# RazorClient/Stark-prover

Measured on AMD Instinct MI355X. Metric: FRI commit field-elems/sec at codeword 2^24; achieved HBM GB/s vs peak, higher is better.
Workload: dtype u32; 1 GPU; fri_commit codeword 2^24, blowup 8 (d=2^21), SHA-256 Merkle per layer, 21 rounds; codeword_log2=24, per_gpu_log2=24, blowup=8, field=p=3*2^30+1, parallelism=single GPU

## Files before the change

stark-prover_amd/csrc/fri_layer.hip:

```cpp
#include <cassert>
#include "fri_internal.hpp"
#include "sha256_fast.hpp"
#include "sha256_quad.hpp"

namespace fri {

#ifdef FRI_STAMPS
#define STAMP_WITH(on, i, fn)                                  \
    do {                                                       \
        if (on) t.st->stamps[t.k][(i)] = fn();                 \
    } while (0)
#else
#define STAMP_WITH(on, i, fn) do {} while (0)
#endif
#define STAMP(on, i) STAMP_WITH(on, i, __builtin_amdgcn_s_memrealtime)
#define STAMP_CLK(on, i) STAMP_WITH(on, i, __builtin_amdgcn_s_memtime)

#ifndef FRI_CHAIN_PRIO
#define FRI_CHAIN_PRIO 3
#endif
__device__ __forceinline__ void chain_prio() {
    if (FRI_CHAIN_PRIO > 0) __builtin_amdgcn_s_setprio(FRI_CHAIN_PRIO);
}

struct Dg { uint32_t w[8]; };

__device__ __forceinline__ void dg_load(const uint32_t* p, Dg& d) {
    uint4 a = reinterpret_cast<const uint4*>(p)[0], b = reinterpret_cast<const uint4*>(p)[1];
    d.w[0] = a.x; d.w[1] = a.y; d.w[2] = a.z; d.w[3] = a.w; d.w[4] = b.x; d.w[5] = b.y; d.w[6] = b.z; d.w[7] = b.w;
}
__device__ __forceinline__ void dg_store(uint32_t* p, const Dg& d) {
    reinterpret_cast<uint4*>(p)[0] = make_uint4(d.w[0], d.w[1], d.w[2], d.w[3]);
    reinterpret_cast<uint4*>(p)[1] = make_uint4(d.w[4], d.w[5], d.w[6], d.w[7]);
}
__device__ __forceinline__ void dg_lds_load(const uint4* p, Dg& d) {
    uint4 a = p[0], b = p[1];
    d.w[0] = a.x; d.w[1] = a.y; d.w[2] = a.z; d.w[3] = a.w; d.w[4] = b.x; d.w[5] = b.y; d.w[6] = b.z; d.w[7] = b.w;
}
__device__ __forceinline__ void dg_lds_store(uint4* p, const Dg& d) {
    p[0] = make_uint4(d.w[0], d.w[1], d.w[2], d.w[3]);
    p[1] = make_uint4(d.w[4], d.w[5], d.w[6], d.w[7]);
}
__device__ __forceinline__ void hnode(const Dg& l, const Dg& r, Dg& o) { shaf::node(l.w, r.w, o.w); }
__device__ __forceinline__ void hleaf(uint32_t v, Dg& o) { shaf::leaf(v, o.w); }
__device__ __forceinline__ void cnode(const Dg& l, const Dg& r, Dg& o) { shaf::node_compact(l.w, r.w, o.w); }
__device__ __forceinline__ void cleaf(uint32_t v, Dg& o) { shaf::leaf_compact(v, o.w); }

__device__ __forceinline__ void pair_level(const uint4* A, uint4* B, uint32_t* out, uint32_t tid, uint32_t cnt,
                                           const shaq::Role& R) {
    if (tid >= max(2 * cnt, 64u)) return;
    const uint32_t q = (tid >> 1) & (cnt - 1), half = (tid & 1u) ^ 1u;
    const bool real = tid < 2 * cnt;
    Dg a, b;
    dg_lds_load(A + 4 * q, a);
    dg_lds_load(A + 4 * q + 2, b);
    uint32_t o[4];
    shaq::node(a.w, b.w, o, R);
    if (!real) return;
    const uint4 v = make_uint4(o[0], o[1], o[2], o[3]);
    B[2 * q + half] = v;
    reinterpret_cast<uint4*>(out + 8 * q)[half] = v;
}

#ifndef FRI_SCHED_PRODUCER
#define FRI_SCHED_PRODUCER 1
#endif
struct SchedLds {
    uint32_t wk[32 * 48];
    uint32_t flag;
};
__device__ __forceinline__ void sched_init(SchedLds* sl) {
    if (FRI_SCHED_PRODUCER && threadIdx.x == 0) sl->flag = 0u;
}
__device__ __forceinline__ void pair_level_s(const uint4* A, uint4* B, uint32_t* out, uint32_t tid, uint32_t cnt,
                                             const shaq::Role& R, SchedLds* sl, uint32_t ord) {
    if (!FRI_SCHED_PRODUCER || cnt > 32) {
        pair_level(A, B, out, tid, cnt, R);
        return;
    }
    const uint32_t wv = tid >> 6;
    if (wv > 1) return;
    const uint32_t lane = tid & 63u;
    const uint32_t q = (lane >> 1) & (cnt - 1), half = (lane & 1u) ^ 1u;
    const bool real = lane < 2 * cnt;
    Dg a, b;
    dg_lds_load(A + 4 * q, a);
    dg_lds_load(A + 4 * q + 2, b);
    if (wv == 1) {
        uint32_t w[16];
#pragma unroll
        for (int i = 0; i < 8; i++) { w[i] = a.w[i]; w[8 + i] = b.w[i]; }
        shaq::produce(w, sl->wk + 48 * q, &sl->flag, 3u * ord, real && (lane & 1u) == 0u, lane == 0u, R);
        return;
    }
    uint32_t o[4];
    shaq::node_ext(a.w, b.w, o, R, sl->wk + 48 * q, &sl->flag, 3u * ord);
    if (!real) return;
    const uint4 v = make_uint4(o[0], o[1], o[2], o[3]);
    B[2 * q + half] = v;
    reinterpret_cast<uint4*>(out + 8 * q)[half] = v;
}

__device__ __forceinline__ void lds_barrier() {
    asm volatile("s_waitcnt lgkmcnt(0)\n\ts_barrier" ::: "memory");
}

__device__ __forceinline__ int wave_max_i(int v) {
#pragma unroll
    for (int off = 32; off > 0; off >>= 1) v = max(v, __shfl_xor(v, off));
    return v;
}

struct Mx3 {
    int m0 = -1, m1 = -1, m2 = -1;
    __device__ __forceinline__ void load(const int32_t* p, uint32_t i) { m0 = p[3 * i]; m1 = p[3 * i + 1]; m2 = p[3 * i + 2]; }
    __device__ __forceinline__ void take(const int32_t* p, uint32_t i) {
        m0 = max(m0, p[3 * i]); m1 = max(m1, p[3 * i + 1]); m2 = max(m2, p[3 * i + 2]);
    }
    __device__ __forceinline__ void store(int32_t* p, uint32_t i) const { p[3 * i] = m0; p[3 * i + 1] = m1; p[3 * i + 2] = m2; }
    __device__ __forceinline__ void wave_max() { m0 = wave_max_i(m0); m1 = wave_max_i(m1); m2 = wave_max_i(m2); }
};
__device__ __forceinline__ void mx3_wave_to_red(Mx3 m, int32_t* red, uint32_t tx) {
    m.wave_max();
    if ((tx & 63) == 0) m.store(red, tx >> 6);
}
__device__ __forceinline__ Mx3 mx3_from_red(const int32_t* red, uint32_t nw) {
    Mx3 m;
    for (uint32_t i = 0; i < nw; i++) m.take(red, i);
    return m;
}
struct Degree { int deg; bool noncanon; };
__device__ __forceinline__ Degree degree_of(int k, const Mx3& m) {
    return {k == 0 ? m.m0 : (m.m1 < 0 ? m.m2 : m.m0), k == 0 && m.m1 >= 0};
}

__device__ __forceinline__ void coef_slice(const LayerTask& t, uint32_t w, uint32_t G, int32_t* red, uint32_t t0,
                                           uint32_t nthr) {
    Mx3 m;
    const uint32_t tx = threadIdx.x - t0;
    const size_t jhi_all = t.jhi ? t.jhi : ~(size_t)0;
    if (t.k == 0) {
        const size_t a = t.jlo, b = min(t.d0, jhi_all), n = b > a ? b - a : 0;
        const size_t cs = (n + G - 1) / G, lo = a + (size_t)w * cs, hi = min(b, lo + cs);
        const uint32_t* in = t.coef_in - t.ibase;
        for (size_t j = lo + tx; j < hi; j += nthr) {
            const uint32_t c = in[j];
            if (c) m.m0 = max(m.m0, (int)j);
            if (c >= P) m.m1 = 0;
        }
    } else {
        const DevState* st = t.st;
        const size_t len = (size_t)(st->deg[t.k - 1] + 1), nlen = (len + 1) / 2;
        const uint32_t beta_m = st->beta_mont[t.k - 1];
        const size_t a = t.jlo, b = min(nlen, jhi_all), n = b > a ? b - a : 0;
        const size_t cs = (n + G - 1) / G, lo = a + (size_t)w * cs, hi = min(b, lo + cs);
        const uint32_t* in = t.coef_in - t.ibase;
        uint32_t* outp = t.coef_out - t.obase;
        for (size_t j = lo + tx; j < hi; j += nthr) {
            uint32_t e = in[2 * j];
            uint32_t o = (2 * j + 1 < len) ? in[2 * j + 1] : 0u;
            uint32_t v = add(e, mmul(o, beta_m));
            outp[j] = v;
            if (v) m.m0 = (int)j;
            if (e) m.m1 = (int)j;
            if (o) m.m2 = (int)j;
        }
    }
    mx3_wave_to_red(m, red, tx);
}
__device__ __forceinline__ void coef_combine(const LayerTask& t, uint32_t w, const int32_t* red, uint32_t nw) {
    mx3_from_red(red, nw).store(t.wgmax, w);
}
__device__ __forceinline__ void coef_task(const LayerTask& t, uint32_t w, uint32_t G, int32_t* red ) {
    coef_slice(t, w, G, red, 0, blockDim.x);
    lds_barrier();
    if (threadIdx.x == 0) coef_combine(t, w, red, blockDim.x / 64);
}

__device__ __forceinline__ void quad(const uint4& vals, uint32_t* lv0, uint32_t* lv1, size_t q ,
                                     Dg& out) {
    Dg a, b, c, d, n0, n1;
    hleaf(vals.x, a); hleaf(vals.y, b); hleaf(vals.z, c); hleaf(vals.w, d);
    dg_store(lv0 + 8 * (4 * q), a); dg_store(lv0 + 8 * (4 * q + 1), b);
    dg_store(lv0 + 8 * (4 * q + 2), c); dg_store(lv0 + 8 * (4 * q + 3), d);
    hnode(a, b, n0);
    hnode(c, d, n1);
    dg_store(lv1 + 8 * (2 * q), n0);
    dg_store(lv1 + 8 * (2 * q + 1), n1);
    hnode(n0, n1, out);
}

template <uint32_t TPB>
__device__ __forceinline__ void lds_two_levels(uint4* lds, const Dg& mine, uint32_t* lv2, uint32_t* lv3, uint32_t* lv4,
                                               size_t g2 ) {
    uint4* A = lds;
    uint4* B = lds + 2 * TPB;
    const uint32_t t = threadIdx.x;
    dg_store(lv2 + 8 * (g2 + t), mine);
    dg_lds_store(A + 2 * t, mine);
    lds_barrier();
    if (t < TPB / 2) {
        Dg l, r, o;
        dg_lds_load(A + 4 * t, l); dg_lds_load(A + 4 * t + 2, r);
        hnode(l, r, o);
        dg_lds_store(B + 2 * t, o);
        dg_store(lv3 + 8 * (g2 / 2 + t), o);
    }
    lds_barrier();
    if (t < TPB / 4) {
        Dg l, r, o;
        dg_lds_load(B + 4 * t, l); dg_lds_load(B + 4 * t + 2, r);
        hnode(l, r, o);
        dg_store(lv4 + 8 * (g2 / 4 + t), o);
    }
}

__device__ __forceinline__ bool gated_off(const LayerTask& t) {
    return t.gst && t.gidx >= 0 && !t.gst->active[t.gidx];
}

__device__ __forceinline__ uint32_t pair_beta(const LayerTask& t) { return t.gst->beta_mont[t.gidx]; }

template <bool FOLD, bool COMMIT, uint32_t TPB, bool PAIR = false>
__global__ __launch_bounds__(TPB) void k_layer_leaf(LayerTask t) {
    if (gated_off(t)) return;
    __shared__ uint4 lds[3 * TPB];
    __shared__ int32_t red[3 * (TPB / 64)];
    const uint32_t L = t.L;
    const size_t wg = PAIR ? (size_t)blockIdx.x + t.wg_base : (size_t)blockIdx.x;
    const size_t q = wg * TPB + threadIdx.x;
    uint4 v;
    if (FOLD) {
        const size_t half = (size_t)1 << L;
        const uint32_t beta_m = COMMIT ? t.st->beta_mont[t.k - 1] : (PAIR ? pair_beta(t) : t.beta_m);
        uint4 a = reinterpret_cast<const uint4*>(t.prev)[q];
        uint4 b = reinterpret_cast<const uint4*>(PAIR ? t.prev2 : t.prev + half)[q];
        uint4 x = reinterpret_cast<const uint4*>(t.xinv)[q];
        v.x = fold_one(a.x, b.x, x.x, beta_m); v.y = fold_one(a.y, b.y, x.y, beta_m);
        v.z = fold_one(a.z, b.z, x.z, beta_m); v.w = fold_one(a.w, b.w, x.w, beta_m);
        reinterpret_cast<uint4*>(t.values)[q] = v;
    } else {
        v = reinterpret_cast<const uint4*>(t.values)[q];
    }
    uint32_t* tr = t.tree;
    Dg top;
    quad(v, tr + 8 * level_offset(L, 0), tr + 8 * level_offset(L, 1), q, top);
    if (COMMIT) coef_task(t, blockIdx.x, gridDim.x, red);
    lds_two_levels<TPB>(lds, top, tr + 8 * level_offset(L, 2), tr + 8 * level_offset(L, 3),
                        tr + 8 * level_offset(L, 4), wg * TPB);
}

#ifndef WIDE_PAIR_MAX
#define WIDE_PAIR_MAX (1u << 16)
#endif

__host__ __device__ __forceinline__ uint32_t wide_levels(uint32_t L) { return L <= 8 + TOP_LOG ? 8u : 4u; }

template <bool FOLD, bool COMMIT, bool PAIR = false>
__global__ __launch_bounds__(256) void k_layer_leaf_wide(LayerTask t) {
    if (gated_off(t)) return;
    STAMP(COMMIT && blockIdx.x == 0 && threadIdx.x == 0, 60);
    __shared__ uint4 lds[2 * 256 + 2 * 128];
    __shared__ int32_t red[12];
    __shared__ SchedLds sl;
    sched_init(&sl);
    const uint32_t L = t.L;
    const size_t wg = PAIR ? (size_t)blockIdx.x + t.wg_base : (size_t)blockIdx.x;
    const size_t grid = PAIR ? (size_t)t.wg_total : (size_t)gridDim.x;
    const size_t i = wg * 256 + threadIdx.x;
    uint32_t v;
    if (FOLD) {
        const size_t half = (size_t)1 << L;
        const uint32_t beta_m = COMMIT ? t.st->beta_mont[t.k - 1] : (PAIR ? pair_beta(t) : t.beta_m);
        v = fold_one(t.prev[i], PAIR ? t.prev2[i] : t.prev[i + half], t.xinv[i], beta_m);
        t.values[i] = v;
    } else {
        v = t.values[i];
    }
    uint32_t* tr = t.tree;
    Dg d;
    cleaf(v, d);
    dg_store(tr + 8 * i, d);
    uint4* A = lds;
    uint4* B = lds + 2 * 256;
    dg_lds_store(A + 2 * threadIdx.x, d);
    lds_barrier();
    STAMP(COMMIT && blockIdx.x == 0 && threadIdx.x == 0, 61);
    uint32_t cnt = 256;
    const shaq::Role qr = shaq::role_of(threadIdx.x);
    if (grid * 128 < WIDE_PAIR_MAX) chain_prio();
    const uint32_t nlev = wide_levels(L);
#pragma unroll 1
    for (uint32_t j = 1; j <= nlev; j++) {
        cnt >>= 1;
        uint32_t* out = tr + 8 * (level_offset(L, j) + (wg << (8 - j)));
        if ((size_t)cnt * grid < WIDE_PAIR_MAX) {
            pair_level_s(A, B, out, threadIdx.x, cnt, qr, &sl, j);
        } else if (threadIdx.x < cnt) {
            Dg a, b, o;
            dg_lds_load(A + 4 * threadIdx.x, a);
            dg_lds_load(A + 4 * threadIdx.x + 2, b);
            hnode(a, b, o);
            dg_lds_store(B + 2 * threadIdx.x, o);
            dg_store(out + 8 * threadIdx.x, o);
        }
        if (COMMIT && j == 2 && threadIdx.x >= 128) coef_slice(t, blockIdx.x, gridDim.x, red, 128, 128);
        lds_barrier();
        uint4* tmp = A; A = B; B = tmp;
    }
    if (COMMIT && threadIdx.x == 128) coef_combine(t, blockIdx.x, red, 2);
    STAMP(COMMIT && blockIdx.x == 0 && threadIdx.x == 0, 62);
}

__device__ __forceinline__ void reduce_mx(const int32_t* in, int32_t* out, uint32_t w, uint32_t R) {
    if (threadIdx.x >= 64) return;
    Mx3 m;
    if (threadIdx.x < R) m.load(in, R * w + threadIdx.x);
    m.wave_max();
    if (threadIdx.x == 0) m.store(out, w);
}

__global__ __launch_bounds__(512) void k_tree_mid(uint32_t* tree, uint32_t L, uint32_t l, const DevState* st,
                                                  int gate, const int32_t* mx_in, int32_t* mx_out, uint32_t R) {
    if (st && gate >= 0 && !st->active[gate]) return;
    constexpr uint32_t NIN = 1024;
    __shared__ uint4 lds[NIN + NIN / 2];
    __shared__ SchedLds sl;
    sched_init(&sl);
    uint4* A = lds;
    uint4* B = lds + NIN;
    const uint32_t t = threadIdx.x;
    const size_t base = (size_t)blockIdx.x * NIN;
    const uint32_t* in = tree + 8 * level_offset(L, l);
    {
        Dg a, b, o;
        dg_load(in + 8 * (base + 2 * t), a);
        dg_load(in + 8 * (base + 2 * t + 1), b);
        if (mx_in) reduce_mx(mx_in, mx_out, blockIdx.x, R);
        hnode(a, b, o);
        dg_lds_store(A + 2 * t, o);
        dg_store(tree + 8 * (level_offset(L, l + 1) + (base >> 1) + t), o);
    }
    lds_barrier();
    const shaq::Role qr = shaq::role_of(t);
    uint32_t cnt = NIN / 2;
#pragma unroll 1
    for (uint32_t j = 2; j <= 4; j++) {
        cnt >>= 1;
        uint32_t* out = tree + 8 * (level_offset(L, l + j) + (base >> j));
        const bool narrow = (size_t)cnt * gridDim.x < WIDE_PAIR_MAX;
        if (narrow) {
            pair_level_s(A, B, out, t, cnt, qr, &sl, j);
        } else if (t < cnt) {
            Dg a, b, o;
            dg_lds_load(A + 4 * t, a);
            dg_lds_load(A + 4 * t + 2, b);
            hnode(a, b, o);
            dg_lds_store(B + 2 * t, o);
            dg_store(out + 8 * t, o);
        }
        lds_barrier();
        uint4* tmp = A; A = B; B = tmp;
    }
}

__global__ __launch_bounds__(256) void k_tree_mid8(uint32_t* tree, uint32_t L, uint32_t l, const DevState* st,
                                                   int gate, const int32_t* mx_in, int32_t* mx_out, uint32_t R) {
    if (st && gate >= 0 && !st->active[gate]) return;
    chain_prio();
    __shared__ uint4 lds[256 + 128];
    __shared__ SchedLds sl;
    sched_init(&sl);
    uint4* A = lds;
    uint4* B = lds + 256;
    const uint32_t t = threadIdx.x;
    const size_t base = (size_t)blockIdx.x * 256;
    const uint32_t* in = tree + 8 * level_offset(L, l);
    const shaq::Role qr = shaq::role_of(t);
    {
        const uint32_t q = t >> 1, half = (t & 1u) ^ 1u;
        Dg a, b;
        dg_load(in + 8 * (base + 2 * q), a);
        dg_load(in + 8 * (base + 2 * q + 1), b);
        if (mx_in) reduce_mx(mx_in, mx_out, blockIdx.x, R);
        uint32_t o[4];
        shaq::node(a.w, b.w, o, qr);
        const uint4 v = make_uint4(o[0], o[1], o[2], o[3]);
        A[2 * q + half] = v;
        reinterpret_cast<uint4*>(tree + 8 * (level_offset(L, l + 1) + (base >> 1) + q))[half] = v;
    }
    lds_barrier();
    uint32_t cnt = 128;
#pragma unroll 1
    for (uint32_t j = 2; j <= 8; j++) {
        cnt >>= 1;
        pair_level_s(A, B, tree + 8 * (level_offset(L, l + j) + (base >> j)), t, cnt, qr, &sl, j);
        lds_barrier();
        uint4* tmp = A; A = B; B = tmp;
    }
}

__device__ __forceinline__ void ktouch(const void* sym) {
    uint32_t a, b, c, d;
    asm volatile("s_nop 4\n\t"
                 "s_load_dword %0, %4, 0x0\n\ts_load_dword %1, %4, 0x40\n\t"
                 "s_load_dword %2, %4, 0x80\n\ts_load_dword %3, %4, 0xc0\n\t"
                 "s_waitcnt lgkmcnt(0)"
                 : "=&s"(a), "=&s"(b), "=&s"(c), "=&s"(d)
                 : "s"(sym)
                 : "memory");
}
__device__ __forceinline__ void kcache_touch_sha_tables() {
    ktouch(&shaf::KTAB[0]);
    ktouch(&shaf::PAD_KW_C.kw[0]);
    ktouch(&shaf::PAD_KW_1024.kw[0]);
    ktouch(&shaf::PAD_KW_1536.kw[0]);
}

__device__ __forceinline__ uint32_t hexch(uint32_t nib) { return nib < 10u ? 0x30u + nib : 0x57u + nib; }
__device__ __forceinline__ void hex2(uint32_t x, uint32_t& hi, uint32_t& lo) {
    hi = (hexch(x >> 28) << 24) | (hexch((x >> 24) & 15u) << 16) | (hexch((x >> 20) & 15u) << 8) | hexch((x >> 16) & 15u);
    lo = (hexch((x >> 12) & 15u) << 24) | (hexch((x >> 8) & 15u) << 16) | (hexch((x >> 4) & 15u) << 8) | hexch(x & 15u);
}
__device__ __forceinline__ uint32_t hexhex(uint32_t b) {
    const uint32_t x = ((b & 0xF0u) << 12) | (b & 0x0Fu);
    const uint32_t ge = ((x + 0x00060006u) >> 4) & 0x00010001u;
    return 0x33303330u + x + ge * 0x2F7u;
}

enum { CJ_REHASH = 0, CJ_MID = 2, CJ_ROOT = 3, CJ_FINAL = 6, CJ_END_ROUND = 6, CJ_END_FINAL = 8 };

__device__ __forceinline__ void chan_job(int j, uint32_t cs[8], uint32_t X[4], uint32_t has, const uint4* root_lds,
                                         uint32_t fv, const shaq::Role& R) {
    j = __builtin_amdgcn_readfirstlane(j);
    has = __builtin_amdgcn_readfirstlane(has);
    uint32_t w[16];
    const bool pad = (j == 1) || (j == 5);
    if (j == 0 || j == 2 || j == 6) {
#pragma unroll
        for (int i = 0; i < 8; i++) hex2(cs[i], w[2 * i], w[2 * i + 1]);
#pragma unroll
        for (int i = 0; i < 4; i++) X[i] = R.iv[i];
    } else if (j == 3 || j == 4) {
        const uint32_t b = (__lane_id() & 15u) + (j == 4 ? 16u : 0u);
        const uint32_t rw = reinterpret_cast<const uint32_t*>(root_lds)[b >> 2];
        const uint32_t hh = hexhex((rw >> (24 - 8 * (b & 3))) & 255u);
#pragma unroll
        for (int jj = 0; jj < 16; jj++) w[jj] = __builtin_amdgcn_readlane(hh, jj);
        if (j == 3 && !has) {
#pragma unroll
            for (int i = 0; i < 4; i++) X[i] = R.iv[i];
        }
    } else if (j == 7) {
#pragma unroll
        for (int i = 0; i < 16; i++) w[i] = 0u;
        w[0] = 0x30303030u; w[1] = 0x30303030u;
        hex2(fv, w[2], w[3]);
        w[4] = 0x80000000u;
        w[15] = 80u * 8u;
    }
    if (pad) shaq::compress_kw(X, j == 1 ? shaf::PAD_KW_C.kw : (has ? shaf::PAD_KW_1536.kw : shaf::PAD_KW_1024.kw), R);
    else shaq::compress(X, w, R);
    if (j == 1 || j == 5 || j == 7) {
#pragma unroll
        for (int i = 0; i < 4; i++) {
            const uint32_t o = shaq::swap01(X[i]);
            cs[i] = R.is_a ? X[i] : o;
            cs[4 + i] = R.is_a ? o : X[i];
        }
    }
}

constexpr uint32_t pow2_32k_mod_p(int k) {
    uint64_t r = 1;
    for (int j = 0; j < k; j++) r = (r << 32) % P;
    return (uint32_t)r;
}
__device__ __forceinline__ uint32_t chan_beta(const uint32_t s[8]) {
    constexpr uint32_t W[8] = {pow2_32k_mod_p(8), pow2_32k_mod_p(7), pow2_32k_mod_p(6), pow2_32k_mod_p(5),
                               pow2_32k_mod_p(4), pow2_32k_mod_p(3), pow2_32k_mod_p(2), pow2_32k_mod_p(1)};
    uint32_t t[8];
#pragma unroll
    for (int i = 0; i < 8; i++) t[i] = mmul(s[i] >= P ? s[i] - P : s[i], W[i]);
    return add(add(add(t[0], t[1]), add(t[2], t[3])), add(add(t[4], t[5]), add(t[6], t[7])));
}


template <typename Value>
__device__ __forceinline__ void leaf_loop(uint32_t N, uint32_t* tr, uint4* A, Value&& value) {
    for (uint32_t i = threadIdx.x; i < max(N, 64u); i += blockDim.x) {
        const uint32_t j = i & (N - 1);
        const bool real = i < N;
        const uint32_t v = value(j, real);
        Dg d;
        cleaf(v, d);
        if (real) {
            dg_store(tr + 8 * j, d);
            dg_lds_store(A + 2 * j, d);
        }
    }
}

__device__ __forceinline__ void level_step(const LayerTask& t, bool stamps, uint32_t it, const uint4* A, uint4* B,
                                           uint32_t* out, uint32_t cnt, const shaq::Role& R, SchedLds* sl,
                                           uint32_t ord) {
    const uint32_t tid = threadIdx.x;
    if (cnt <= 128) {
        STAMP_CLK(stamps && it < 18 && tid == 0, 24 + 2 * it);
        pair_level_s(A, B, out, tid, cnt, R, sl, ord);
        STAMP_CLK(stamps && it < 18 && tid == 0, 25 + 2 * it);
        return;
    }
#pragma unroll 1
    for (uint32_t q = tid; q < cnt; q += blockDim.x) {
        Dg a, b, o;
        dg_lds_load(A + 4 * q, a);
        dg_lds_load(A + 4 * q + 2, b);
#ifdef FRI_STAMPS
        if (stamps && it < 18 && q == 0) asm volatile("s_waitcnt lgkmcnt(0)" ::: "memory");
#endif
        STAMP_CLK(stamps && it < 18 && q == 0, 24 + 2 * it);
        cnode(a, b, o);
        STAMP_CLK(stamps && it < 18 && q == 0, 25 + 2 * it);
        dg_lds_store(B + 2 * q, o);
        dg_store(out + 8 * q, o);
    }
}

__device__ __forceinline__ int chan_drain(const LayerTask& t, int job, int job_end, bool level, uint32_t cnt,
                                           uint32_t cs[8], uint32_t X[4], uint32_t has, const uint4* root_lds,
                                           uint32_t fv, const shaq::Role& R) {
    if (job >= job_end || (level && !(cnt <= 192 && job < CJ_ROOT))) return job;
    do {
        STAMP(threadIdx.x == 448 && job == CJ_ROOT, 14);
        STAMP(threadIdx.x == 448 && job == CJ_ROOT + 2, 13);
        chan_job(job, cs, X, has, root_lds, fv, R);
        STAMP(threadIdx.x == 448 && job >= CJ_ROOT && job <= CJ_ROOT + 2, 20 + job - CJ_ROOT);
        job++;
    } while (!level && job < job_end);
    return job;
}

struct RoundOut { uint32_t active, beta_m; };
__device__ __forceinline__ RoundOut layer_results(const LayerTask& t, const Degree& dg, const uint32_t cs[8],
                                                  uint32_t fv, uint32_t fbeta1, const uint4* root_lds) {
    DevState* st = t.st;
    const int k = t.k, deg = dg.deg;
    if (dg.noncanon) {
        st->active[k] = 0;
        st->status = 1u;
        return {0u, 0u};
    }
    st->deg[k] = deg;
    Dg root;
    dg_lds_load(root_lds, root);
#pragma unroll
    for (int i = 0; i < 8; i++) st->roots[k][i] = root.w[i];
    st->n_layers = (uint32_t)k + 1;
    STAMP(true, 15);
    if (deg >= 1 && k < MAXR && t.L >= 1) {
        uint32_t beta = chan_beta(cs);
#pragma unroll
        for (int i = 0; i < 8; i++) st->chan[i] = cs[i];
        st->chan_has = 1;
        st->chan_pending = 1;
        if (fbeta1) beta = fbeta1 - 1u;
        st->beta[k] = beta;
        const uint32_t bm = to_mont(beta);
        st->beta_mont[k] = bm;
        st->active[k] = 1;
        st->n_rounds = (uint32_t)k + 1;
        STAMP(true, 16);
        return {1u, bm};
    }
    st->active[k] = 0;
    if (deg >= 1) { st->status = 7u; return {0u, 0u}; }
#pragma unroll
    for (int i = 0; i < 8; i++) st->chan[i] = cs[i];
    st->final_value = fv;
    st->final_degree = deg;
    st->chan_has = 1;
    st->chan_pending = 0;
    return {0u, 0u};
}

template <bool FROM_LEAVES, bool COMMIT, bool SHARD = false>
__global__ __launch_bounds__(512) void k_tree_top(LayerTask t, uint32_t l, const int32_t* mx, uint32_t G) {
    static_assert(!(FROM_LEAVES && (COMMIT || SHARD)), "from the leaves: standalone trees only");
    if (gated_off(t)) return;
    chain_prio();
    __shared__ uint4 lds[2 * 1024 + 2 * 512];
    __shared__ int32_t red[24];
    __shared__ SchedLds sl;
    sched_init(&sl);
    const uint32_t L = t.L;
    const uint32_t N = 1u << (L - l);
    const uint32_t tid = threadIdx.x;

    const bool chan_wave = COMMIT && tid >= 448;
    DevState* st = t.st;
    uint32_t cs[8], X[4];
    uint32_t has = 0, fbeta1 = 0;
    int job = CJ_END_FINAL;
    if (chan_wave) {
#pragma unroll
        for (int i = 0; i < 8; i++) cs[i] = st->chan[i];
        const uint32_t h = st->chan_has, pend = st->chan_pending;
        const uint32_t fo = COMMIT ? st->forced : 0u, fb = st->forced_beta[t.k < MAXR ? t.k : 0];
        has = h;
        job = !h ? CJ_ROOT : (pend ? CJ_REHASH : CJ_MID);
        if (fo && t.k < MAXR) fbeta1 = fb + 1u;
    }
    if (tid >= 384 && tid < 448) kcache_touch_sha_tables();
    uint4* A = lds;
    uint4* B = lds + 2 * 1024;
    uint32_t* tr = t.tree;
    STAMP(COMMIT && tid == 0, 0);
    if (FROM_LEAVES) {
        leaf_loop(N, tr, A, [&](uint32_t j, bool) { return t.values[j]; });
    } else if (SHARD && COMMIT) {
        const ShardTop& sh = *t.shard;
        for (uint32_t i = tid; i < N; i += blockDim.x) {
            Dg d;
            dg_load(sh.recs_in + REC_WORDS * sh.rank_of_block[i], d);
            dg_lds_store(A + 2 * i, d);
            dg_store(tr + 8 * i, d);
        }
        Mx3 m;
        if (tid < sh.G) {
            m.load(reinterpret_cast<const int32_t*>(sh.recs_in + REC_WORDS * tid + 8), 0);
            if (sh.sched_on) { m.m0 = sh.sched_deg; m.m1 = t.k == 0 ? -1 : 0; m.m2 = -1; }
        }
        mx3_wave_to_red(m, red, tid);
    } else {
        const uint32_t* in = tr + 8 * level_offset(L, l);
        Mx3 m;
        if (COMMIT && tid < G) m.load(mx, tid);
        for (uint32_t i = tid; i < N; i += blockDim.x) {
            Dg d;
            dg_load(in + 8 * i, d);
            dg_lds_store(A + 2 * i, d);
        }
        if (SHARD && !COMMIT) {
            const ShardTop& sh = *t.shard;
            for (uint32_t i = tid; i < sh.rec_R; i += blockDim.x) m.take(sh.rec_mx, i);
            mx3_wave_to_red(m, red, tid);
        }
        if (COMMIT) {
            for (uint32_t i = tid + blockDim.x; i < G; i += blockDim.x) m.take(mx, i);
            mx3_wave_to_red(m, red, tid);
        }
    }
    lds_barrier();
    const Degree dg = COMMIT ? degree_of(t.k, mx3_from_red(red, 8)) : Degree{-1, false};
    const bool is_final = COMMIT && dg.deg < 1;
    const int job_end = is_final ? CJ_END_FINAL : CJ_END_ROUND;
    uint32_t fv = 0;
    if (chan_wave && is_final && dg.deg == 0)
        fv = SHARD ? t.shard->recs_in[11] : (t.k == 0 ? t.coef_in : t.coef_out)[0];
    STAMP(COMMIT && tid == 0, 1);
    STAMP_CLK(COMMIT && tid == 0, 17);
    const uint32_t nlev = L - l;
    const uint32_t total = nlev + (COMMIT ? 1u : 0u);
    const shaq::Role R = shaq::role_of(tid);
    uint32_t cnt = N;
#pragma unroll 1
    for (uint32_t it = 0; it < total; it++) {
        const bool level = it < nlev;
        if (level) {
            cnt >>= 1;
            level_step(t, COMMIT, it, A, B, tr + 8 * level_offset(L, l + 1 + it), cnt, R, &sl, it);
        }
        if (chan_wave) job = chan_drain(t, job, job_end, level, cnt, cs, X, has, A, fv, R);
        lds_barrier();
        if (level) {
            uint4* tmp = A; A = B; B = tmp;
            STAMP(COMMIT && tid == 0 && it < 11, 2 + it);
            STAMP_CLK(COMMIT && tid == 0 && it + 1 == nlev, 18);
            STAMP(COMMIT && tid == 0 && it + 1 == nlev, 19);
        }
    }
    if (SHARD && !COMMIT && tid == 448) {
        const ShardTop& sh = *t.shard;
        const Mx3 m = mx3_from_red(red, 8);
        Dg root;
        dg_lds_load(A, root);
        uint32_t* rec = sh.rec_out;
        dg_store(rec, root);
        reinterpret_cast<uint4*>(rec)[2] = make_uint4((uint32_t)m.m0, (uint32_t)m.m1, (uint32_t)m.m2, sh.rec_c0[0]);
        reinterpret_cast<uint4*>(rec)[3] = make_uint4(0u, 0u, 0u, 0u);
    }
    if (COMMIT && tid == 448) layer_results(t, dg, cs, fv, fbeta1, A);
}

struct TailTask {
    LayerTask t[TAIL_LOG + 1];
    uint32_t n;
};

template <bool FOLD0>
__global__ __launch_bounds__(512) void k_tree_tail(TailTask tt) {
    const LayerTask& t0 = tt.t[0];
    if (gated_off(t0)) return;
    chain_prio();
    constexpr uint32_t NMAX = 1u << TAIL_LOG;
    __shared__ uint4 lds[2 * NMAX + NMAX];
    __shared__ uint32_t vals[2][NMAX];
    __shared__ uint32_t coefs[2][NMAX];
    __shared__ int32_t red[24];
    __shared__ uint32_t s_beta_m, s_active;
    __shared__ int32_t s_deg;
    __shared__ uint32_t s_fbeta[TAIL_LOG + 2];
    __shared__ uint32_t xv[2 * NMAX];
    __shared__ SchedLds sl;
    sched_init(&sl);
    uint32_t ord = 0;
    const uint32_t tid = threadIdx.x;
    const bool chan_wave = tid >= 448;
    DevState* st = t0.st;
    auto prefetch_x = [&](uint32_t t0p, uint32_t nthr) {
        uint32_t off = 1u << tt.t[0].L;
        for (uint32_t li = 1; li < tt.n; li++) {
            const uint32_t N = 1u << tt.t[li].L;
            for (uint32_t j = tid - t0p; j < N; j += nthr) xv[off + j] = tt.t[li].xinv[j];
            off += N;
        }
    };
    uint32_t cs[8], X[4];
    uint32_t has = 0;
    if (chan_wave) {
#pragma unroll
        for (int i = 0; i < 8; i++) cs[i] = st->chan[i];
        has = st->chan_has;
    }
    uint32_t pending = chan_wave ? st->chan_pending : 0u;
    if (tid >= 384 && tid < 448) kcache_touch_sha_tables();
    if (tid < tt.n + 1) {
        const int kk = t0.k + (int)tid;
        s_fbeta[tid] = (st->forced && kk < MAXR) ? st->forced_beta[kk] + 1u : 0u;
    }
    uint32_t beta_m = FOLD0 ? st->beta_mont[t0.k - 1] : 0u;
    int prev_deg = FOLD0 ? st->deg[t0.k - 1] : -1;
    const shaq::Role R = shaq::role_of(tid);
    uint32_t xoff = 0;
#pragma unroll 1
    for (uint32_t li = 0; li < tt.n; li++) {
        const LayerTask& t = tt.t[li];
        const int k = t.k;
        const uint32_t L = t.L, N = 1u << L;
        const uint32_t* xl = li ? xv + xoff : t.xinv;
        xoff += N;
        const bool fold = FOLD0 || li > 0;
        uint32_t* cur_v = vals[li & 1];
        const uint32_t* prev_v = vals[(li & 1) ^ 1];
        uint32_t* cur_c = coefs[li & 1];
        const uint32_t* prev_c = coefs[(li & 1) ^ 1];
        uint4* A = lds;
        uint4* B = lds + 2 * NMAX;
        uint32_t* tr = t.tree;
        STAMP(tid == 0, 0);
        leaf_loop(N, tr, A, [&](uint32_t j, bool real) {
            uint32_t v;
            if (fold) {
                const uint32_t a = li ? prev_v[j] : t.prev[j], b = li ? prev_v[j + N] : t.prev[j + N];
                v = fold_one(a, b, xl[j], beta_m);
                if (real) t.values[j] = v;
            } else {
                v = t.values[j];
            }
            if (real) cur_v[j] = v;
            return v;
        });
        const uint32_t nlev = L;
        const uint32_t coef_it = N > 256 ? 1u : 0u;
        const bool coef_late = nlev > coef_it;
        auto coef_fold = [&](uint32_t t0c, uint32_t nthr) {
            Mx3 m;
            const uint32_t tx = tid - t0c;
            if (k == 0) {
                for (size_t j = tx; j < t.d0; j += nthr) {
                    const uint32_t c = t.coef_in[j];
                    if (c) m.m0 = max(m.m0, (int)j);
                    if (c >= P) m.m1 = 0;
                }
            } else {
                const uint32_t len = (uint32_t)(prev_deg + 1), nlen = (len + 1) / 2;
                const bool in_lds = li > 0 && k >= 2;
                for (uint32_t j = tx; j < nlen; j += nthr) {
                    const uint32_t e = in_lds ? prev_c[2 * j] : t.coef_in[2 * j];
                    const uint32_t o = (2 * j + 1 < len) ? (in_lds ? prev_c[2 * j + 1] : t.coef_in[2 * j + 1]) : 0u;
                    const uint32_t v = add(e, mmul(o, beta_m));
                    cur_c[j] = v;
                    if (v) m.m0 = (int)j;
                    if (e) m.m1 = (int)j;
                    if (o) m.m2 = (int)j;
                }
            }
            mx3_wave_to_red(m, red, tx);
        };
        if (!coef_late) coef_fold(0, blockDim.x);
        if (li == 0 && !coef_late) prefetch_x(0, blockDim.x);
        lds_barrier();
        STAMP(tid == 0, 1);
        STAMP_CLK(tid == 0, 17);
        Degree dg{1, false};
        int job_end = CJ_END_ROUND;
        uint32_t fv = 0;
        auto settle = [&](uint32_t nw) {
            dg = degree_of(k, mx3_from_red(red, nw));
            job_end = dg.deg < 1 ? CJ_END_FINAL : CJ_END_ROUND;
            if (chan_wave && dg.deg == 0) fv = (k == 0) ? t.coef_in[0] : cur_c[0];
        };
        if (!coef_late) settle(8);
        int job = CJ_END_FINAL;
        if (chan_wave) job = !has ? CJ_ROOT : (pending ? CJ_REHASH : CJ_MID);
        const uint32_t total = nlev + 1;
        uint32_t cnt = N;
#pragma unroll 1
        for (uint32_t it = 0; it < total; it++) {
            const bool level = it < nlev;
            if (level) {
                cnt >>= 1;
                level_step(t, true, it, A, B, tr + 8 * level_offset(L, 1 + it), cnt, R, &sl, ord++);
            }
            if (chan_wave) job = chan_drain(t, job, job_end, level, cnt, cs, X, has, A, fv, R);
            if (coef_late && it == coef_it && tid >= 256 && tid < 384) coef_fold(256, 128);
            if (li == 0 && coef_late && it == coef_it && tid >= 384 && tid < 448) prefetch_x(384, 64);
            lds_barrier();
            if (coef_late && it == coef_it) settle(2);
            if (level) {
                uint4* tmp = A; A = B; B = tmp;
                STAMP(tid == 0 && it < 11, 2 + it);
                STAMP_CLK(tid == 0 && it + 1 == nlev, 18);
                STAMP(tid == 0 && it + 1 == nlev, 19);
            }
        }
        if (tid == 448) {
            const RoundOut r = layer_results(t, dg, cs, fv, s_fbeta[li], A);
            s_beta_m = r.beta_m;
            s_active = r.active;
            s_deg = dg.deg;
        }
        if (chan_wave) { has = 1; pending = 1; }
        lds_barrier();
        if (!s_active) break;
        beta_m = s_beta_m;
        prev_deg = s_deg;
    }
}

static LayerTask with_gate(const LayerTask& in) {
    LayerTask t = in;
    if (t.st) { t.gst = t.st; t.gidx = t.k > 0 ? t.k - 1 : -1; }
    return t;
}

#ifndef QUAD_TPB
#define QUAD_TPB 512
#endif
#ifndef QUAD_MIN_LOG
#define QUAD_MIN_LOG 19
#endif

template <typename KernelLaunch>
static void pair_parts(LayerTask t, uint32_t G, hipStream_t s, const std::function<void()>& after_part1,
                       KernelLaunch&& go) {
    t.wg_total = G;
    if (!after_part1) {
        t.wg_base = 0;
        go(t, G);
        return;
    }
    const uint32_t h = G / 2;
    t.wg_base = t.send_half ? h : 0u;
    go(t, h);
    after_part1();
    t.wg_base = t.send_half ? 0u : h;
    go(t, h);
}

void launch_layer(const LayerTask& tin, hipStream_t s, hipEvent_t ev_leaf_end, const std::function<void()>& after_leaf,
                  hipEvent_t ev_before_top, const std::function<void()>& after_part1) {
    const LayerTask t = with_gate(tin);
    const uint32_t L = t.L;
    const bool fold = t.prev != nullptr;
    const bool commit = t.st != nullptr;
    const bool pair = t.prev2 != nullptr;
    const int32_t* nomx = nullptr;
    static_assert(TAIL_LOG == TOP_LOG, "every commit layer the top could take from its leaves goes to launch_tail");
    if (L <= TOP_LOG) {
        assert(!fold && !commit);
        hipLaunchKernelGGL((k_tree_top<true, false>), dim3(1), dim3(512), 0, s, t, 0u, nomx, 1u);
        if (ev_leaf_end) hipEventRecord(ev_leaf_end, s);
        return;
    }
    uint32_t G, out_per_wg;
    if (L >= QUAD_MIN_LOG) {
        constexpr uint32_t TPB = QUAD_TPB;
        G = (uint32_t)(((size_t)1 << L) / (4 * TPB));
        out_per_wg = TPB / 4;
        if (pair) {
            pair_parts(t, G, s, after_part1, [&](const LayerTask& tp, uint32_t g) {
                hipLaunchKernelGGL((k_layer_leaf<true, false, TPB, true>), dim3(g), dim3(TPB), 0, s, tp);
            });
        } else if (fold) {
            if (commit) hipLaunchKernelGGL((k_layer_leaf<true, true, TPB>), dim3(G), dim3(TPB), 0, s, t);
            else hipLaunchKernelGGL((k_layer_leaf<true, false, TPB>), dim3(G), dim3(TPB), 0, s, t);
        } else {
            if (commit) hipLaunchKernelGGL((k_layer_leaf<false, true, TPB>), dim3(G), dim3(TPB), 0, s, t);
            else hipLaunchKernelGGL((k_layer_leaf<false, false, TPB>), dim3(G), dim3(TPB), 0, s, t);
        }
    } else {
        G = 1u << (L - 8);
        out_per_wg = 256u >> wide_levels(L);
        if (pair) {
            pair_parts(t, G, s, after_part1, [&](const LayerTask& tp, uint32_t g) {
                hipLaunchKernelGGL((k_layer_leaf_wide<true, false, true>), dim3(g), dim3(256), 0, s, tp);
            });
        } else if (fold) {
            if (commit) hipLaunchKernelGGL((k_layer_leaf_wide<true, true>), dim3(G), dim3(256), 0, s, t);
            else hipLaunchKernelGGL((k_layer_leaf_wide<true, false>), dim3(G), dim3(256), 0, s, t);
        } else {
            if (commit) hipLaunchKernelGGL((k_layer_leaf_wide<false, true>), dim3(G), dim3(256), 0, s, t);
            else hipLaunchKernelGGL((k_layer_leaf_wide<false, false>), dim3(G), dim3(256), 0, s, t);
        }
    }
    if (ev_leaf_end) hipEventRecord(ev_leaf_end, s);
    if (after_leaf) after_leaf();
    const int gate = t.gidx;
    const int32_t* mx = commit ? t.wgmax : nullptr;
    size_t mx_off = 3 * (size_t)G;
    uint32_t l = L >= QUAD_MIN_LOG ? 4u : wide_levels(L);
    while (L - l > TOP_LOG) {
        const size_t nodes = (size_t)1 << (L - l);
        const bool eight = nodes < ((size_t)1 << 18);
        assert(!eight || L - l >= 8 + 6);
        const uint32_t nin = eight ? 256u : 1024u;
        const uint32_t grid = (uint32_t)(nodes / nin);
        const uint32_t R = nin / out_per_wg;
        int32_t* mx_out = commit ? t.wgmax + mx_off : nullptr;
        if (eight)
            hipLaunchKernelGGL(k_tree_mid8, dim3(grid), dim3(256), 0, s, t.tree, L, l, t.gst, gate, mx, mx_out, R);
        else
            hipLaunchKernelGGL(k_tree_mid, dim3(grid), dim3(512), 0, s, t.tree, L, l, t.gst, gate, mx, mx_out, R);
        if (commit) { mx = mx_out; mx_off += 3 * (size_t)grid; }
        G = grid;
        out_per_wg = eight ? 1u : nin / 16;
        l += eight ? 8u : 4u;
    }
    if (ev_before_top) hipStreamWaitEvent(s, ev_before_top, 0);
    if (commit) hipLaunchKernelGGL((k_tree_top<false, true>), dim3(1), dim3(512), 0, s, t, l, mx, G);
    else if (t.shard) hipLaunchKernelGGL((k_tree_top<false, false, true>), dim3(1), dim3(512), 0, s, t, l, nomx, G);
    else hipLaunchKernelGGL((k_tree_top<false, false>), dim3(1), dim3(512), 0, s, t, l, nomx, G);
}

void launch_tail(const LayerTask* ts, uint32_t n, hipStream_t s) {
    TailTask tt{};
    tt.n = n;
    for (uint32_t i = 0; i < n; i++) tt.t[i] = ts[i];
    tt.t[0] = with_gate(ts[0]);
    if (ts[0].prev) hipLaunchKernelGGL((k_tree_tail<true>), dim3(1), dim3(512), 0, s, tt);
    else hipLaunchKernelGGL((k_tree_tail<false>), dim3(1), dim3(512), 0, s, tt);
}

__global__ __launch_bounds__(256) void k_coef(LayerTask t) {
    if (gated_off(t)) return;
    __shared__ int32_t red[12];
    coef_task(t, blockIdx.x, gridDim.x, red);
}

void launch_coef(const LayerTask& tin, uint32_t G, hipStream_t s) {
    const LayerTask t = with_gate(tin);
    hipLaunchKernelGGL(k_coef, dim3(G), dim3(256), 0, s, t);
}

void launch_top(const LayerTask& tin, uint32_t l, const int32_t* mx, uint32_t G, hipStream_t s) {
    const LayerTask t = with_gate(tin);
    if (t.shard) hipLaunchKernelGGL((k_tree_top<false, true, true>), dim3(1), dim3(512), 0, s, t, l, mx, G);
    else hipLaunchKernelGGL((k_tree_top<false, true>), dim3(1), dim3(512), 0, s, t, l, mx, G);
}

}
```

Before: 3.649 billion field-elems/s.

## Add register-climb tree kernel for mid Merkle levels with 18-20 remaining depth

```diff
diff --git a/stark-prover_amd/csrc/fri_layer.hip b/stark-prover_amd/csrc/fri_layer.hip
--- a/stark-prover_amd/csrc/fri_layer.hip
+++ b/stark-prover_amd/csrc/fri_layer.hip
@@ -849,6 +849,92 @@
     }
 }
 
+template <uint32_t R, typename Beside>
+__device__ __forceinline__ void climb_regs(uint32_t* tree, uint32_t L, uint32_t l, size_t n0 ,
+                                           Dg& top, Beside&& while_loading) {
+    const uint32_t* in = tree + 8 * (level_offset(L, l) + n0);
+    if constexpr (R == 0) {
+        dg_load(in, top);
+        while_loading();
+        return;
+    }
+    constexpr uint32_t NP = R ? 1u << (R - 1) : 1u;
+    Dg na, nb, a, b, cur;
+    Dg left[R + 1];
+    dg_load(in, na);
+    dg_load(in + 8, nb);
+    while_loading();
+    uint32_t p = 0, lev = 1;
+#pragma unroll 1
+    for (uint32_t i = 0; i + 1 < (1u << R); i++) {
+        if (lev == 1) {
+            a = na;
+            b = nb;
+            if (p + 1 < NP) {
+                dg_load(in + 16 * (p + 1), na);
+                dg_load(in + 16 * (p + 1) + 8, nb);
+            }
+        } else {
+#pragma unroll
+            for (uint32_t j = 1; j < R; j++)
+                if (lev == j + 1) a = left[j];
+            b = cur;
+        }
+        hnode(a, b, cur);
+        const uint32_t idx = p >> (lev - 1);
+        uint32_t* out = tree + 8 * (level_offset(L, l + lev) + (n0 >> lev) + idx);
+        if (lev == R) {
+            dg_store(out, cur);
+        } else if (idx & 1u) {
+#pragma unroll
+            for (uint32_t j = 1; j < R; j++)
+                if (lev == j) dg_store(out - 8, left[j]);
+            dg_store(out, cur);
+            lev++;
+        } else {
+#pragma unroll
+            for (uint32_t j = 1; j < R; j++)
+                if (lev == j) left[j] = cur;
+            p++;
+            lev = 1;
+        }
+    }
+    top = cur;
+}
+
+constexpr uint32_t CLIMB_LOG_TPB = 10, CLIMB_TPB = 1u << CLIMB_LOG_TPB, CLIMB_LOG_GRID = 8;
+
+template <uint32_t R>
+__global__ __launch_bounds__(CLIMB_TPB) void k_tree_climb(LayerTask t, uint32_t l, const int32_t* mx_in, int32_t* mx_out,
+                                                          uint32_t RP ) {
+    if (gated_off(t)) return;
+    constexpr uint32_t LT = CLIMB_LOG_TPB, TPB = CLIMB_TPB;
+    __shared__ uint4 lds[2 * TPB + TPB];
+    __shared__ SchedLds sl;
+    sched_init(&sl);
+    const uint32_t tid = threadIdx.x, w = blockIdx.x, L = t.L;
+    if (tid >= TPB - 64) kcache_touch_sha_tables();
+    Dg top;
+    climb_regs<R>(t.tree, L, l, (((size_t)w << LT) + tid) << R, top, [&] {
+        if (mx_in) reduce_mx(mx_in, mx_out, w, RP);
+    });
+    uint4* A = lds;
+    uint4* B = lds + 2 * TPB;
+    dg_lds_store(A + 2 * tid, top);
+    lds_barrier();
+    chain_prio();
+    const shaq::Role qr = shaq::role_of(tid);
+    uint32_t cnt = TPB;
+#pragma unroll 1
+    for (uint32_t it = 0; it < LT; it++) {
+        cnt >>= 1;
+        level_step(t, false, it, A, B, t.tree + 8 * (level_offset(L, l + R + 1 + it) + (size_t)w * cnt), cnt, qr, &sl,
+                   it);
+        lds_barrier();
+        uint4* tmp = A; A = B; B = tmp;
+    }
+}
+
 static LayerTask with_gate(const LayerTask& in) {
     LayerTask t = in;
     if (t.st) { t.gst = t.st; t.gidx = t.k > 0 ? t.k - 1 : -1; }
@@ -861,6 +947,8 @@
 #ifndef QUAD_MIN_LOG
 #define QUAD_MIN_LOG 19
 #endif
+
+static uint32_t mid_levels(uint32_t D) { return D >= 21 ? 4u : D >= 18 ? D - CLIMB_LOG_GRID : 8u; }
 
 template <typename KernelLaunch>
 static void pair_parts(LayerTask t, uint32_t G, hipStream_t s, const std::function<void()>& after_part1,
@@ -932,21 +1020,29 @@
     size_t mx_off = 3 * (size_t)G;
     uint32_t l = L >= QUAD_MIN_LOG ? 4u : wide_levels(L);
     while (L - l > TOP_LOG) {
-        const size_t nodes = (size_t)1 << (L - l);
-        const bool eight = nodes < ((size_t)1 << 18);
-        assert(!eight || L - l >= 8 + 6);
-        const uint32_t nin = eight ? 256u : 1024u;
+        const uint32_t D = L - l;
+        const size_t nodes = (size_t)1 << D;
+        const uint32_t up = mid_levels(D);
+        assert(D >= 14 && (up == 4 ? D >= 21 : D - up >= 6 && D - up <= TOP_LOG));
+        const size_t nin = (size_t)1 << (up == 4 ? 10u : up);
         const uint32_t grid = (uint32_t)(nodes / nin);
-        const uint32_t R = nin / out_per_wg;
+        const uint32_t R = (uint32_t)(nin / out_per_wg);
+        assert(R <= 64);
         int32_t* mx_out = commit ? t.wgmax + mx_off : nullptr;
-        if (eight)
+        if (up == 8)
             hipLaunchKernelGGL(k_tree_mid8, dim3(grid), dim3(256), 0, s, t.tree, L, l, t.gst, gate, mx, mx_out, R);
+        else if (up == 4)
+            hipLaunchKernelGGL(k_tree_mid, dim3(grid), dim3(512), 0, s, t.tree, L, l, t.gst, gate, mx, mx_out, R);
+        else if (D == 18)
+            hipLaunchKernelGGL(k_tree_climb<0>, dim3(grid), dim3(CLIMB_TPB), 0, s, t, l, mx, mx_out, R);
+        else if (D == 19)
+            hipLaunchKernelGGL(k_tree_climb<1>, dim3(grid), dim3(CLIMB_TPB), 0, s, t, l, mx, mx_out, R);
         else
-            hipLaunchKernelGGL(k_tree_mid, dim3(grid), dim3(512), 0, s, t.tree, L, l, t.gst, gate, mx, mx_out, R);
+            hipLaunchKernelGGL(k_tree_climb<2>, dim3(grid), dim3(CLIMB_TPB), 0, s, t, l, mx, mx_out, R);
         if (commit) { mx = mx_out; mx_off += 3 * (size_t)grid; }
         G = grid;
-        out_per_wg = eight ? 1u : nin / 16;
-        l += eight ? 8u : 4u;
+        out_per_wg = up == 4 ? 64u : 1u;
+        l += up;
     }
     if (ev_before_top) hipStreamWaitEvent(s, ev_before_top, 0);
     if (commit) hipLaunchKernelGGL((k_tree_top<false, true>), dim3(1), dim3(512), 0, s, t, l, mx, G);
```

Result: no change. 3.654 billion field-elems/s, median of 2 (+0.1%).
